# bhavyageethika/multimodal_autonomous_driving_perception_and_planning

Hardware: AMD Instinct MI355X
Metric: end-to-end frames/sec (1280x720 synthetic) (higher is better)
Workload: dtype f64; 1 GPU; config4: 64 stream(s)/GPU x 1-frame window per step, 1280x720, simulated detection + IoU tracker + 6-state KF + 21-candidate planner, one launch per step, up to 4 consecutive steps in flight; streams_per_gpu=64, window=1, graph=False, taggers=False, allgather_track_tables=False, fused_step=True, overlapped_steps=4, steps_per_library_call=8, parallelism=stream-sharded x1

## Files before the change

multimodal_autonomous_driving_perception_and_planning_amd/csrc/common.h:

```cpp
#pragma once
#include <hip/hip_runtime.h>

#include <cstdarg>
#include <cstdio>
#include <vector>

#include "avhot.h"

struct PlannerTables;

struct av_ctx {
    int device = -1;
    int n_cus = 256;
    hipStream_t side = nullptr;
    hipEvent_t ev_fork = nullptr, ev_join = nullptr;
    bool planner_ready = false;
    av_planner_cfg pcfg{};
    int n_points = 0, n_lat = 0, n_cand = 0;
    double* d_ptab = nullptr;
    double* d_cdf = nullptr;
    void* d_simtab = nullptr;
    std::vector<hipGraphExec_t> graphs;
    void* lane = nullptr;
    void* yolo = nullptr;
};

void av_set_error(const char* fmt, ...);

#define AV_HIP(expr)                                                                          \
    do {                                                                                      \
        hipError_t e_ = (expr);                                                               \
        if (e_ != hipSuccess) {                                                               \
            av_set_error("%s:%d: %s -> %s", __FILE__, __LINE__, #expr, hipGetErrorString(e_)); \
            return AV_EHIP;                                                                   \
// ... 136 lines not shown
```

multimodal_autonomous_driving_perception_and_planning_amd/csrc/planner.hip:

```cpp
#include "common.h"

#include <cmath>



namespace {

struct PlanParams {
    int n, n_lat, C;
    double dt, H;
    double w_lat, w_vel, w_acc, w_curv;
    const double *t, *alpha, *q, *dtd, *lat;
    double atq[20];
};

static const double ATAN_Q[20] = {
    -0x1.5555555555549p-2, 0x1.99999999979b9p-3,  -0x1.24924923e22b4p-3, 0x1.c71c718e5a102p-4,
    -0x1.745d120df88fbp-4, 0x1.3b1362fc35ab5p-4,  -0x1.110deef367776p-4, 0x1.e1b3c8d50e91fp-5,
    -0x1.ae2c7119eb922p-5, 0x1.81fdd2525246ap-5,  -0x1.56daf4786fd80p-5, 0x1.2575526b2309ap-5,
    -0x1.d168e01adf666p-6, 0x1.462cc26bda000p-6,  -0x1.8055065b73333p-7, 0x1.693bd6b79999ap-8,
    -0x1.fdf4e15cccccdp-10, 0x1.f224118000000p-12, -0x1.2568700000000p-14, 0x1.2ed799999999ap-18,
};

__device__ __forceinline__ double atan2_fast(double y, double x, const double (&Q)[20]) {
// ... 83 lines not shown
}
__device__ __forceinline__ void rank_and_store(const double* cc, int C, int c, int f, double* __restrict__ cost,
                                               int32_t* __restrict__ order) {
    const double mine = cc[c];
    int rank = 0;
    for (int o2 = 0; o2 < C; ++o2) {
        const double v = cc[o2];
        rank += (v < mine || (v == mine && o2 < c)) ? 1 : 0;
    }
    cost[(size_t)f * C + c] = mine;
    order[(size_t)f * C + rank] = c;
}

struct PlanNoHook {
    __device__ __forceinline__ void operator()(int) const {}
};

struct PlanLists {
    const double* ref; int n_ref;
    const double* obs; int n_obs;
};
struct PlanShared {
    static constexpr int OSTRIDE = 3;
    static constexpr bool MOVING = false;
    const double* ref; int n_ref;
    const double* obs; int n_obs;
    __device__ __forceinline__ PlanLists at(int) const { return PlanLists{ref, n_ref, obs, n_obs}; }
    __device__ __forceinline__ bool has_ref(int) const { return n_ref > 0; }
};
template <int OS>
struct PlanEachT {
// ... 14 lines not shown
            const int pth = f / ref_stride;
            l.n_ref = path_points(pth);
            l.ref = ref + (size_t)pth * rcap * 2;
        }
        if (obs) {
            const int k = n_obs[f];
            l.n_obs = k < 0 ? 0 : (k > ocap ? ocap : k);
            l.obs = obs + (size_t)f * ocap * OS;
        }
        return l;
    }
};
using PlanEach = PlanEachT<3>;
using PlanEachMoving = PlanEachT<5>;

template <int G, int NW, class Hook = PlanNoHook, class Lists = PlanShared>
__device__ __forceinline__ void plan_block_lists(const PlanParams& p, int f0, int n_states, const double* __restrict__ state,
                                                 const Lists lists, double* __restrict__ wp, double* __restrict__ cost,
                                                 int32_t* __restrict__ order, double* sm, int state_f0 = -1, int rot = 0,
                                                 Hook after1 = Hook()) {
    const int n = p.n, C = p.C;
    const int sd = state_f0 < 0 ? 0 : state_f0 - f0;
    double* vs = sm;
    double* base = vs + (size_t)G * 3 * n * 2;
    double* trig = base + even_up(G * 3 * 3);
    double* costs = trig + G * 8;
    double* stage_all = costs + 3 * even_up(G * C);
    const int CS = even_up(G * C);

    const int tid = threadIdx.x, lane = tid & 63;
    double* stage = stage_all + (size_t)(tid >> 6) * n * 6;
    const int wid = ((tid >> 6) + NW - rot) % NW;
    constexpr int P = G * 3;
    static_assert(NW >= 2, "the heading terms take the last wave");

    auto bcast = [&](double x, int i) {
        const unsigned lo = (unsigned)__builtin_amdgcn_readlane((int)(unsigned)__double_as_longlong(x), i);
        const unsigned hi = (unsigned)__builtin_amdgcn_readlane((int)(unsigned)((unsigned long long)__double_as_longlong(x) >> 32), i);
        return __longlong_as_double((long long)(((unsigned long long)hi << 32) | lo));
    };
    auto terms = [&](double v0, double dv, int i, double& v, double& vdt, double& velt, double& acct) {
        v = blend_velocity(v0, dv, p.alpha[i]);
        vdt = v * p.dt;
        velt = velocity_term(p.w_vel, v);
        acct = 0.0;
        if (i > 0)
            acct = acceleration_term(p.w_acc, v, blend_velocity(v0, dv, p.alpha[i - 1]), p.dtd[i]);
    };
    auto cost_chains = [&](double velt, double acct, unsigned long long hasm, double* b) {
        double sv = 0.0;
#pragma unroll
        for (int i = 0; i < 64; ++i)
            if (i < n) sv = sv + bcast(velt, i);
        double run = sv, sa = 0.0;
#pragma unroll
        for (int i = 1; i < 64; ++i)
            if (i < n && ((hasm >> i) & 1ull)) {
                const double term = bcast(acct, i);
                run = run + term, sa = sa + term;
            }
        if (lane == 0) b[0] = sv, b[1] = sa, b[2] = run;
    };

    const bool fast = n <= 64 && P <= NW;
    double k_velt = 0.0, k_acct = 0.0;
    unsigned long long k_has = 0;
    bool k_live = false;
    if (fast) {
        if (wid < P) {
            const int g = wid / 3, k = wid - g * 3, f = f0 + g;
            if (f < n_states) {
                const double v0 = state[(size_t)(f + sd) * 4 + 3];
                const double dv = target_speed(k) - v0;
                double* o = vs + ((size_t)(g * 3 + k) * n) * 2;
                double v = 0.0, vdt = 0.0;
                bool has = false;
                if (lane < n) terms(v0, dv, lane, v, vdt, k_velt, k_acct), has = lane > 0 && p.dtd[lane] > 0.0;
                k_has = __ballot(has), k_live = true;
                double sacc = 0.0, my_s = 0.0;
#pragma unroll
                for (int i = 1; i < 64; ++i)
                    if (i < n) {
                        sacc = sacc + bcast(vdt, i);
                        my_s = lane == i ? sacc : my_s;
                    }
                if (lane < n) o[2 * lane] = v, o[2 * lane + 1] = my_s;
            }
        }
    } else {
        for (int pr = wid; pr < P; pr += NW) {
            const int g = pr / 3, k = pr - g * 3, f = f0 + g;
            if (f >= n_states) continue;
// ... 7 lines not shown
                terms(v0, dv, i, v, vdt, velt, acct);
                o[2 * i] = v, tv[i] = vdt, tv[n + i] = velt, tv[2 * n + i] = acct;
            }
            wave_lds_fence();
            if (lane == 0) {
                double sacc = 0.0, sv = 0.0;
                o[1] = 0.0;
                sv = sv + tv[n];
                for (int i = 1; i < n; ++i) {
                    sacc = sacc + tv[i];
                    o[2 * i + 1] = sacc;
                    sv = sv + tv[n + i];
                }
                double run = sv, sa = 0.0;
                for (int i = 1; i < n; ++i) {
                    if (p.dtd[i] > 0.0) {
                        const double term = tv[2 * n + i];
                        run = run + term, sa = sa + term;
                    }
                }
                b[0] = sv, b[1] = sa, b[2] = run;
            }
            wave_lds_fence();
        }
    }
    if (wid == NW - 1 && lane < 2 * G) {
        const int g = lane >> 1, f = f0 + g;
        if (f < n_states) {
            const double h0 = state[(size_t)(f + sd) * 4 + 2];
            double* tg = trig + g * 8;
            double sn, cs;
            if (lane & 1) {
                sincos(h0 + 1.5707963267948966, &sn, &cs);
                tg[4] = cs, tg[5] = sn;
            } else {
                sincos(h0, &sn, &cs);
                tg[0] = state[(size_t)(f + sd) * 4 + 0], tg[1] = state[(size_t)(f + sd) * 4 + 1];
                tg[2] = cs, tg[3] = sn, tg[6] = h0;
            }
        }
    }
    __syncthreads();
    if (k_live) cost_chains(k_velt, k_acct, k_has, base + wid * 3);
    after1(wid);

    const double q_l = lane < n ? p.q[lane] : 0.0, q_l1 = lane + 1 < n ? p.q[lane + 1] : 0.0, t_l = lane < n ? p.t[lane] : 0.0;
    for (int j = fast ? (wid - P % NW + NW) % NW : wid; j < G * C; j += NW) {
        const int g = j / C, c = j - g * C, f = f0 + g;
        if (f >= n_states) continue;
        const PlanLists ls = lists.at(f);
        const double* ref = ls.ref;
        const double* obs = ls.obs;
        const int n_ref = ls.n_ref, n_obs = ls.n_obs;
        const bool extra = n_ref > 0 || n_obs > 0;
        const int li = c / 3, k = c - li * 3;
        const double df = p.lat[li];
        const double* tg = trig + g * 8;
        const PlanFrame fr{tg[0], tg[1], tg[2], tg[3], tg[4], tg[5]};
        const double h0 = tg[6];
        const double* o = vs + ((size_t)(g * 3 + k) * n) * 2;

        for (int i = lane; i < n; i += 64) {
            const double v = o[2 * i], s = o[2 * i + 1];
            const bool first = i == lane;
            double x, y, hd = 0.0;
            fr.point(s, df * (first ? q_l : p.q[i]), x, y);
            if (i < n - 1) {
                double x1, y1;
                fr.point(o[2 * i + 3], df * (first ? q_l1 : p.q[i + 1]), x1, y1);
                hd = atan2_fast(y1 - y, x1 - x, p.atq);
            }
            double* w = stage + (size_t)i * 6;
            w[0] = x, w[1] = y, w[2] = hd, w[3] = v, w[4] = first ? t_l : p.t[i], w[5] = 0.0;
        }
        wave_lds_fence();
        double lat_sum = 0.0, curv_sum = 0.0, obs_sum = 0.0;
        for (int i = lane; i < n; i += 64) {
            double* w = stage + (size_t)i * 6;
            double curv = 0.0;
            if (i > 0 && i < n - 1) w[5] = curv = tile_curvature(stage, i, p.dt);
            curv_sum += p.w_curv * (curv * curv);
            const double x = w[0], y = w[1];
            if (n_ref > 0) lat_sum += ref_path_term(p.w_lat, ref, n_ref, x, y);
            for (int q = 0; q < n_obs; ++q)
                add_obstacle_penalty<Lists::MOVING>(obs_sum, obs + Lists::OSTRIDE * q, x, y, w[4]);
        }
        wave_lds_fence();
        if (lane == 0) tile_last_heading(stage, n, h0);
        curv_sum = wave_sum_dpp(curv_sum);
        if (extra) lat_sum = wave_sum_dpp(lat_sum), obs_sum = wave_sum_dpp(obs_sum);
        if (lane == 0) costs[g * C + c] = lat_sum, costs[CS + g * C + c] = curv_sum, costs[2 * CS + g * C + c] = obs_sum;
        wave_lds_fence();
        if (wp) {
            const double2* src = reinterpret_cast<const double2*>(stage);
            double2* dst = reinterpret_cast<double2*>(wp + ((size_t)f * C + c) * n * 6);
            for (int q = lane; q < n * 3; q += 64) dst[q] = src[q];
        }
        wave_lds_fence();
    }
    __syncthreads();

    for (int idx = tid; idx < G * C; idx += NW * 64) {
        const int g = idx / C, c = idx - g * C, k = c % 3;
        const double* b = base + (g * 3 + k) * 3;
        const bool with_ref = lists.has_ref(f0 + g < n_states ? f0 + g : f0);
        const double va = with_ref ? (costs[idx] + b[0]) + b[1] : b[2];
        const double total = (va + costs[CS + idx]) + costs[2 * CS + idx];
        costs[idx] = total;
    }
    __syncthreads();
    for (int idx = tid; idx < G * C; idx += NW * 64) {
        const int g = idx / C, c = idx - g * C, f = f0 + g;
        if (f >= n_states) continue;
        rank_and_store(costs + g * C, C, c, f, cost, order);
    }
}

template <int G, int NW, class Hook = PlanNoHook>
__device__ __forceinline__ void plan_block(const PlanParams& p, int f0, int n_states, const double* state, const double* ref, int n_ref,
                                           const double* obs, int n_obs, double* wp, double* cost, int32_t* order, double* sm,
                                           int state_f0 = -1, int rot = 0, Hook after1 = Hook()) {
    plan_block_lists<G, NW, Hook, PlanShared>(p, f0, n_states, state, PlanShared{ref, n_ref, obs, n_obs}, wp, cost, order, sm, state_f0,
                                              rot, after1);
}

template <int G, int NW, class Lists = PlanShared>
__global__ void __launch_bounds__(NW * 64) planner_kernel(PlanParams p, int n_states, const double* __restrict__ state, Lists lists,
                                                          double* __restrict__ wp, double* __restrict__ cost,
                                                          int32_t* __restrict__ order) {
    extern __shared__ __attribute__((aligned(16))) double sm[];
    plan_block_lists<G, NW, PlanNoHook, Lists>(p, blockIdx.x * G, n_states, state, lists, wp, cost, order, sm);
}

template <int FPW, bool EXTRA, class Lists = PlanShared>
__global__ void __launch_bounds__(256) planner_wave_kernel(PlanParams p, int n_states,
                                                           const double* __restrict__ state, Lists lists,
                                                           double* __restrict__ wp, double* __restrict__ cost,
                                                           int32_t* __restrict__ order) {
// ... 476 lines not shown
```

multimodal_autonomous_driving_perception_and_planning_amd/csrc/step.hip:

```cpp
#define AVHOT_DEVICE_ONLY
#include "simdet.hip"
#include "tracker.hip"
#include "kf.hip"
#include "planner.hip"
#undef AVHOT_DEVICE_ONLY

namespace {

struct StepArgs {
    int S, h, w, dcap, tcap;
    av_tracker_cfg tcfg;
    av_kf_cfg kcfg;
    PlanParams pp;
    int32_t* frame_count; const SimRow* tab; const double* cdf;
    int32_t *det_n, *det_box, *det_cls; double* det_conf; int32_t* det_status;
    unsigned char* trk_state; av_track_row* snap; int32_t* snap_n; int32_t* det2trk;
    const double* z; double *kf_state, *vstate, *plan_state;
    double *wp, *cost; int32_t* order;
    uint8_t* wire; int stream0, frame0;
    int* flags; int seq, spin, fence, stage_off;
};

constexpr int STEP_NW = 8;

// ... 9 lines not shown
        if (!on) return;
        const unsigned long long n = __builtin_amdgcn_s_memrealtime();
        atomicAdd(acc + k, n - t);
        t = n;
    }
};

__device__ void StepClock::start(const StepArgs& a, int role) {
    on = a.flags && (a.fence & 8) && threadIdx.x == 0;
    if (!on) return;
    acc = reinterpret_cast<unsigned long long*>(a.flags + flag_stats(a.S)) + role * 16;
    t = __builtin_amdgcn_s_memrealtime();
    atomicAdd(acc + 15, 1ull);
}

__device__ __forceinline__ bool seq_enter(const StepArgs& a, int slot, int* go) {
    if (threadIdx.x == 0) {
        int ok = 0;
        int* const counter = a.flags + 32 * slot;
        int* const fault = a.flags + flag_fault(a.S);
        const int want = a.seq, spin = a.spin;
        for (int n = 0; n <= spin; ++n) {
            if ((int)((unsigned)__hip_atomic_load(counter, __ATOMIC_RELAXED, __HIP_MEMORY_SCOPE_AGENT) - (unsigned)want) >= 0) { ok = 1; break; }
            if ((n & 255) == 255 && __hip_atomic_load(fault, __ATOMIC_RELAXED, __HIP_MEMORY_SCOPE_AGENT) != 0) break;
        }
        if (!ok) atomicOr(a.flags + flag_fault(a.S), 1);
        if (ok && (a.fence & 8) && a.seq != 0) {
            const unsigned long long tp = __hip_atomic_load(reinterpret_cast<unsigned long long*>(a.flags + 32 * slot + 2), __ATOMIC_RELAXED,
                                                            __HIP_MEMORY_SCOPE_AGENT);
            const unsigned long long now = __builtin_amdgcn_s_memrealtime();
// ... 10 lines not shown
__device__ __forceinline__ void seq_leave(const StepArgs& a, int slot) {
    if (a.fence & 2) __builtin_amdgcn_fence(__ATOMIC_RELEASE, "agent");
    if (a.fence & 8)
        __hip_atomic_store(reinterpret_cast<unsigned long long*>(a.flags + 32 * slot + 2), __builtin_amdgcn_s_memrealtime(), __ATOMIC_RELAXED,
                           __HIP_MEMORY_SCOPE_AGENT);
    __hip_atomic_store(a.flags + 32 * slot, (int)((unsigned)a.seq + 1u), __ATOMIC_RELAXED, __HIP_MEMORY_SCOPE_AGENT);
}
__device__ __forceinline__ void fetch_record(const void* src, void* dst_lds, int n8, int first, int end, bool coherent) {
    unsigned long long* g = const_cast<unsigned long long*>(reinterpret_cast<const unsigned long long*>(src));
    unsigned long long* l = reinterpret_cast<unsigned long long*>(dst_lds);
    if ((int)threadIdx.x < first || (int)threadIdx.x >= end) return;
    for (int i = (int)threadIdx.x - first; i < n8; i += end - first)
        l[i] = coherent ? __hip_atomic_load(g + i, __ATOMIC_RELAXED, __HIP_MEMORY_SCOPE_AGENT) : g[i];
}

template <int PW>
__global__ void __launch_bounds__(PW * 64) hot_step_kernel(StepArgs a) {
    extern __shared__ __attribute__((aligned(16))) unsigned char smem[];
    __shared__ int go, fc_stage;
    __shared__ __attribute__((aligned(16))) double kf_stage[AV_KF_STATE_DOUBLES + 2];
    __shared__ __attribute__((aligned(32))) double kf_start[4];
    __shared__ __attribute__((aligned(16))) double kf_carry[KF_CARRY_DOUBLES];
    __shared__ int kf_tail;
    __shared__ __attribute__((aligned(16))) int d_box[8 * 4];
    __shared__ __attribute__((aligned(16))) double d_conf[8], d_area[8], z_stage[4];
    __shared__ int d_cls[8], d_n[1];
    const int tid = threadIdx.x;
    const bool seq = a.flags != nullptr;
    if ((int)blockIdx.x < a.S) {
        if (PW > STEP_NW && tid >= STEP_NW * 64) return;
        const int s = blockIdx.x;
        StepClock ck;
        ck.start(a, 0);
        int fc_before = 0;
        if (tid == 0) {
            fc_before = seq ? (int)((unsigned)a.flags[flag_base(a.S) + s] + (unsigned)a.seq) : a.frame_count[s];
            fc_stage = fc_before;
            simdet_frame<true>(0, 0, 0, a.h, a.w, a.dcap, &fc_stage, a.tab, a.cdf, d_n, d_box, d_cls, d_conf,
                               a.det_status ? a.det_status + s : nullptr);
            for (int i = 0; i < a.dcap; ++i)
                d_area[i] = (double)(d_box[4 * i + 2] - d_box[4 * i]) * (double)(d_box[4 * i + 3] - d_box[4 * i + 1]);
        }
        ck.mark(0);
        if (seq && !seq_enter(a, 2 * s, &go)) return;
        ck.mark(1);
        unsigned char* stage = smem + a.stage_off;
        int fc0 = 0;
        if (seq && tid == 0) fc0 = __hip_atomic_load(a.frame_count + s, __ATOMIC_RELAXED, __HIP_MEMORY_SCOPE_AGENT);
        fetch_record(a.trk_state + (size_t)s * state_bytes(a.tcap, a.tcfg.trajectory_length), stage,
                     (HDR_INTS * 4 + a.tcap * (int)sizeof(av_track_row)) / 8, 64, STEP_NW * 64, seq);
        if (tid == 0) {
            if (seq) {
                if (fc0 != fc_before) atomicOr(a.flags + flag_fault(a.S), 2);
                __hip_atomic_store(a.frame_count + s, fc_stage, __ATOMIC_RELAXED, __HIP_MEMORY_SCOPE_AGENT);
            } else {
                a.frame_count[s] = fc_stage;
            }
        }
        if (seq) __builtin_amdgcn_s_waitcnt(0x0F70);
        __syncthreads();
        ck.mark(2);
        if (tid < a.dcap) {
            reinterpret_cast<int4*>(a.det_box)[(size_t)s * a.dcap + tid] = reinterpret_cast<const int4*>(d_box)[tid];
            a.det_cls[(size_t)s * a.dcap + tid] = d_cls[tid];
            a.det_conf[(size_t)s * a.dcap + tid] = d_conf[tid];
            if (tid == 0) a.det_n[s] = d_n[0];
        }
        tracker_body<false, 8, STEP_NW>(a.tcfg, 1, a.dcap, d_n, d_box, d_cls, d_conf, a.tcap, a.trk_state, a.snap, a.snap_n,
                                        a.det2trk, 1, s, smem, 0xFEDCBA9876543210ull, stage, seq, 0,
                                        seq ? a.flags + 32 * (2 * s) : nullptr, (int)((unsigned)a.seq + 1u), (a.fence & 8) != 0, d_area);
        ck.mark(3);
        if (a.wire) {
            __syncthreads();
            if (tid < a.tcap)
                wire_put(a.wire + (size_t)s * (AV_WIRE_HDR_BYTES + (size_t)a.tcap * AV_WIRE_ROW_BYTES), tid, a.snap_n[s], a.tcap,
                         a.snap + (size_t)s * a.tcap, a.stream0 + s, a.frame0 + fc_stage);
        }
    } else {
        const int s = blockIdx.x - a.S;
        StepClock ck;
        ck.start(a, 1);
        if (tid < 4) z_stage[tid] = a.z[(size_t)s * 4 + tid];
        if (seq && !seq_enter(a, 2 * s + 1, &go)) return;
        ck.mark(1);
        double *vs = a.vstate + (size_t)s * AV_VSTATE_DOUBLES, *ps = a.plan_state + (size_t)s * 4;
        if (tid < 64) {
            double* rec = a.kf_state + (size_t)s * AV_KF_STATE_DOUBLES;
            fetch_record(rec, kf_stage, AV_KF_STATE_DOUBLES, 0, 64, seq);
            __builtin_amdgcn_fence(__ATOMIC_RELEASE, "workgroup", "local");
            __builtin_amdgcn_wave_barrier();
            __builtin_amdgcn_fence(__ATOMIC_ACQUIRE, "workgroup", "local");
            ck.mark(2);
            const bool separable = kf_axis_chain1(a.kcfg, z_stage, kf_stage, kf_start, kf_carry, tid);
            if (tid == 0) {
                kf_tail = separable;
                if (!separable) {
                    kf_dense_stream_lds(a.kcfg, 0, 1, z_stage, nullptr, kf_stage, vs, kf_start);
                    *reinterpret_cast<double4*>(ps) = *reinterpret_cast<const double4*>(kf_start);
                }
            }
            __builtin_amdgcn_fence(__ATOMIC_RELEASE, "workgroup", "local");
            __builtin_amdgcn_wave_barrier();
            __builtin_amdgcn_fence(__ATOMIC_ACQUIRE, "workgroup", "local");
            if (tid < AV_KF_STATE_DOUBLES) {
                if (seq)
                    __hip_atomic_store(reinterpret_cast<unsigned long long*>(rec) + tid, (unsigned long long)__double_as_longlong(kf_stage[tid]),
                                       __ATOMIC_RELAXED, __HIP_MEMORY_SCOPE_AGENT);
                else
                    rec[tid] = kf_stage[tid];
            }
        }
        ck.mark(3);
        __syncthreads();
        ck.mark(4);
        constexpr int KF_ROT = 4;
        static_assert(KF_ROT + 3 < PW, "wave 0 must not be a phase-1 pair wave nor the heading wave (task wave PW - 1)");
        if (seq && tid < 64) {
            __builtin_amdgcn_s_waitcnt(0x0F70);
            if (tid == 0) seq_leave(a, 2 * s + 1);
        }
        ck.mark(5);
        const bool clocks = seq && (a.fence & 8);
        auto tail = [&](int task_wave) {
            if (task_wave != 0 || !kf_tail) return;
            const unsigned long long t0 = clocks ? __builtin_amdgcn_s_memrealtime() : 0ull;
            kf_axis_tail1(a.kcfg, kf_stage, kf_carry, vs, ps, tid & 63);
            if (clocks && (tid & 63) == 0)
                atomicAdd(reinterpret_cast<unsigned long long*>(a.flags + flag_stats(a.S)) + 16 + 7, __builtin_amdgcn_s_memrealtime() - t0);
        };
        plan_block<1, PW>(a.pp, s, a.S, kf_start, nullptr, 0, nullptr, 0, a.wp, a.cost, a.order, reinterpret_cast<double*>(smem), 0, KF_ROT,
                          tail);
        ck.mark(6);
    }
}

}

static size_t hot_step_tracker_lds(int dcap, int tcap, int& stage_off) {
    static_assert(STEP_NW == 8, "tracker_lds_bytes sizes the replica kernel's eight column waves");
    const size_t lds_t = (tracker_lds_bytes(tcap, dcap, 1, true, 0) + 15) & ~size_t(15);
    stage_off = (int)lds_t;
    return lds_t + HDR_INTS * 4 + (size_t)tcap * sizeof(av_track_row);
}

static size_t hot_step_static_lds(const void* kernel) {
    hipFuncAttributes fa{};
    return hipFuncGetAttributes(&fa, kernel) == hipSuccess ? (size_t)fa.sharedSizeBytes : (size_t)16384;
}

static int hot_step_shape(const av_ctx* ctx, int n_streams, size_t lds_t, int depth, size_t& lds_out, int& pw_out) {
    static const size_t lds_static16 = hot_step_static_lds(reinterpret_cast<const void*>(hot_step_kernel<16>));
    static const size_t lds_static8 = hot_step_static_lds(reinterpret_cast<const void*>(hot_step_kernel<8>));
    const char* pwe = getenv("AVHOT_STEP_PW");
    int pw = pwe && atoi(pwe) == 8 ? 8 : 16;
    size_t lds = 0;
    for (;;) {
        const size_t lds_p = plan_lds_doubles(1, ctx->n_points, ctx->n_cand, pw) * 8;
        lds = lds_t > lds_p ? lds_t : lds_p;
        const size_t lds_static = pw == 16 ? lds_static16 : lds_static8;
        if (lds + lds_static > 64 * 1024) {
            AV_REQUIRE(pw == 16 && !pwe, AV_EINVAL,
                       "av_hot_step: configuration needs %zu B of dynamic + %zu B of static LDS (limit 65536)", lds, lds_static);
            pw = 8;
            continue;
        }
        if (depth <= 1) break;
        int per_cu = 0;
        if (pw == 16) AV_HIP(hipOccupancyMaxActiveBlocksPerMultiprocessor(&per_cu, hot_step_kernel<16>, 16 * 64, lds));
        else AV_HIP(hipOccupancyMaxActiveBlocksPerMultiprocessor(&per_cu, hot_step_kernel<8>, 8 * 64, lds));
        if ((long long)depth * 2 * n_streams <= (long long)per_cu * ctx->n_cus) break;
        AV_REQUIRE(pw == 16 && !pwe, AV_EINVAL, "av_hot_step: %d launches of %d workgroups in flight do not fit the device (%d per CU x %d CUs)",
                   depth, 2 * n_streams, per_cu, ctx->n_cus);
        pw = 8;
    }
    lds_out = lds, pw_out = pw;
    return AV_OK;
}

static int hot_step_args(av_ctx* ctx, const av_tracker_cfg* tcfg, const av_kf_cfg* kcfg, int n_streams, int h,
                           int w, int dcap, int tcap, int32_t* frame_count, int32_t* det_n, int32_t* det_box, int32_t* det_cls,
                           double* det_conf, int32_t* det_status, void* tracker_state, av_track_row* snap, int32_t* snap_n,
                           int32_t* det2trk, const double* z, double* kf_state, double* vstate, double* plan_state,
                           double* waypoints, double* cost, int32_t* order, void* wire, int stream0, int frame0, int32_t* seq_flags,
                           int seq, StepArgs& a, size_t& lds_out, int& pw_out, int depth = 1) {
    AV_REQUIRE(ctx && tcfg && kcfg && frame_count && det_n && det_box && det_cls && det_conf && tracker_state && z && kf_state &&
                   vstate && plan_state && cost && order,
               AV_EINVAL, "av_hot_step: null argument");
    AV_REQUIRE(n_streams > 0, AV_EINVAL, "av_hot_step: n_streams must be > 0");
    AV_REQUIRE(ctx->planner_ready && ctx->d_simtab, AV_ESTATE, "av_hot_step: call av_planner_configure first");
    AV_REQUIRE((snap == nullptr) == (snap_n == nullptr), AV_EINVAL, "av_hot_step: snap and snap_n go together");
    AV_REQUIRE(!wire || snap, AV_EINVAL, "av_hot_step: the wire tables are made from the snapshot rows");
    AV_REQUIRE(tcap == 64 && dcap >= 7 && dcap <= 8 && tcfg->iou_threshold > 0.0 && tcfg->trajectory_length >= 1, AV_EINVAL,
               "av_hot_step: needs tcap 64, dcap 7..8 and iou_threshold > 0 (use the stage calls otherwise)");
    AV_REQUIRE(h > 0 && w > 121, AV_EINVAL, "av_hot_step: frame %dx%d too small", w, h);
    a = StepArgs{};
    a.S = n_streams, a.h = h, a.w = w, a.dcap = dcap, a.tcap = tcap;
    a.tcfg = *tcfg, a.kcfg = *kcfg;
    fill_params(ctx, a.pp);
    a.frame_count = frame_count, a.tab = (const SimRow*)ctx->d_simtab, a.cdf = ctx->d_cdf;
    a.det_n = det_n, a.det_box = det_box, a.det_cls = det_cls, a.det_conf = det_conf, a.det_status = det_status;
    a.trk_state = (unsigned char*)tracker_state, a.snap = snap, a.snap_n = snap_n, a.det2trk = det2trk;
    a.z = z, a.kf_state = kf_state, a.vstate = vstate, a.plan_state = plan_state;
    a.wp = waypoints, a.cost = cost, a.order = order;
    a.wire = (uint8_t*)wire, a.stream0 = stream0, a.frame0 = frame0;
    a.flags = seq_flags, a.seq = seq;
    const char* spe = seq_flags ? getenv("AVHOT_STEP_SPIN") : nullptr;
    a.spin = spe ? atoi(spe) : (1 << 22);
    const char* fe = seq_flags ? getenv("AVHOT_STEP_FENCE") : nullptr;
    a.fence = fe ? atoi(fe) : 0;
    int stage_off = 0;
    const size_t lds_t = hot_step_tracker_lds(dcap, tcap, stage_off);
    a.stage_off = stage_off;
    return hot_step_shape(ctx, n_streams, lds_t, depth, lds_out, pw_out);
}

static int hot_step_go(const StepArgs& a, size_t lds, int pw, av_stream_t stream) {
    if (pw == 16) hipLaunchKernelGGL(hot_step_kernel<16>, dim3(2 * a.S), dim3(16 * 64), lds, as_stream(stream), a);
    else hipLaunchKernelGGL(hot_step_kernel<8>, dim3(2 * a.S), dim3(8 * 64), lds, as_stream(stream), a);
    AV_LAUNCH_CHECK();
    return AV_OK;
}

static int hot_step_launch(av_ctx* ctx, av_stream_t stream, const av_tracker_cfg* tcfg, const av_kf_cfg* kcfg, int n_streams, int h,
                           int w, int dcap, int tcap, int32_t* frame_count, int32_t* det_n, int32_t* det_box, int32_t* det_cls,
                           double* det_conf, int32_t* det_status, void* tracker_state, av_track_row* snap, int32_t* snap_n,
                           int32_t* det2trk, const double* z, double* kf_state, double* vstate, double* plan_state,
                           double* waypoints, double* cost, int32_t* order, void* wire, int stream0, int frame0, int32_t* seq_flags,
                           int seq, int depth = 1) {
    StepArgs a;
    size_t lds;
    int pw;
    const int rc = hot_step_args(ctx, tcfg, kcfg, n_streams, h, w, dcap, tcap, frame_count, det_n, det_box, det_cls, det_conf, det_status,
                                 tracker_state, snap, snap_n, det2trk, z, kf_state, vstate, plan_state, waypoints, cost, order, wire, stream0,
                                 frame0, seq_flags, seq, a, lds, pw, depth);
    return rc != AV_OK ? rc : hot_step_go(a, lds, pw, stream);
}

extern "C" int av_hot_step_fits(av_ctx* ctx, int n_streams, int dcap, int tcap, int depth) {
    AV_REQUIRE(ctx && n_streams > 0 && depth >= 1, AV_EINVAL, "av_hot_step_fits: bad argument");
    AV_REQUIRE(ctx->planner_ready, AV_ESTATE, "av_hot_step_fits: call av_planner_configure first");
    AV_REQUIRE(tcap == 64 && dcap >= 7 && dcap <= 8, AV_EINVAL, "av_hot_step_fits: needs tcap 64, dcap 7..8");
    AV_HIP(hipSetDevice(ctx->device));
    int stage_off = 0;
    size_t lds = 0;
    int pw = 0;
    return hot_step_shape(ctx, n_streams, hot_step_tracker_lds(dcap, tcap, stage_off), depth, lds, pw);
}

extern "C" int av_hot_step(av_ctx* ctx, av_stream_t stream, const av_tracker_cfg* tcfg, const av_kf_cfg* kcfg, int n_streams, int h,
                           int w, int dcap, int tcap, int32_t* frame_count, int32_t* det_n, int32_t* det_box, int32_t* det_cls,
                           double* det_conf, int32_t* det_status, void* tracker_state, av_track_row* snap, int32_t* snap_n,
                           int32_t* det2trk, const double* z, double* kf_state, double* vstate, double* plan_state,
                           double* waypoints, double* cost, int32_t* order, void* wire, int stream0, int frame0) {
    return hot_step_launch(ctx, stream, tcfg, kcfg, n_streams, h, w, dcap, tcap, frame_count, det_n, det_box, det_cls, det_conf, det_status,
                           tracker_state, snap, snap_n, det2trk, z, kf_state, vstate, plan_state, waypoints, cost, order, wire, stream0,
                           frame0, nullptr, 0);
}

extern "C" int av_hot_step_seq(av_ctx* ctx, av_stream_t stream, const av_tracker_cfg* tcfg, const av_kf_cfg* kcfg, int n_streams, int h,
                               int w, int dcap, int tcap, int32_t* frame_count, int32_t* det_n, int32_t* det_box, int32_t* det_cls,
                               double* det_conf, int32_t* det_status, void* tracker_state, av_track_row* snap, int32_t* snap_n,
// ... 7 lines not shown
                           frame0, seq_flags, seq, depth);
}

extern "C" int av_hot_steps_seq(av_ctx* ctx, int depth, const av_stream_t* streams, const av_tracker_cfg* tcfg, const av_kf_cfg* kcfg,
                                int n_streams, int h, int w, int dcap, int tcap, int32_t* frame_count, int32_t* det_status,
                                void* tracker_state, double* kf_state, const av_step_set* sets, const double* z_steps, void* wire_steps,
                                int stream0, int frame0, int32_t* seq_flags, int seq0, int n_steps) {
    AV_REQUIRE(seq_flags && n_steps > 0 && sets && streams, AV_EINVAL, "av_hot_steps_seq: bad argument");
    AV_REQUIRE(depth >= 2 && depth <= AV_STEP_MAX_DEPTH, AV_EINVAL, "av_hot_steps_seq: depth %d not in [2, %d]", depth, AV_STEP_MAX_DEPTH);
    for (int k = 0; k < depth; ++k)
        for (int j = 0; j < k; ++j)
            AV_REQUIRE(streams[k] != streams[j], AV_EINVAL, "av_hot_steps_seq: the %d steps in flight need %d different HIP streams", depth, depth);
    StepArgs par[AV_STEP_MAX_DEPTH];
    size_t lds = 0;
    int pw = 16;
    for (int k = 0; k < depth; ++k) {
        const av_step_set& b = sets[k];
        const int rc = hot_step_args(ctx, tcfg, kcfg, n_streams, h, w, dcap, tcap, frame_count, b.det_n, b.det_box, b.det_cls, b.det_conf, det_status,
                                     tracker_state, b.snap, b.snap_n, b.det2trk, z_steps ? z_steps : b.z, kf_state, b.vstate, b.plan_state,
                                     b.waypoints, b.cost, b.order, wire_steps, stream0, frame0, seq_flags, seq0, par[k], lds, pw, depth);
        if (rc != AV_OK) return rc;
    }
    const size_t zb = (size_t)n_streams * 4, wb = (size_t)n_streams * (AV_WIRE_HDR_BYTES + (size_t)tcap * AV_WIRE_ROW_BYTES);
    for (int i = 0; i < n_steps; ++i) {
        const int q = (int)((unsigned)seq0 + (unsigned)i), k = (int)((unsigned)q % (unsigned)depth);
        StepArgs& a = par[k];
        a.seq = q;
        if (z_steps) a.z = z_steps + (size_t)i * zb;
        if (wire_steps) a.wire = (uint8_t*)wire_steps + (size_t)i * wb;
        const int rc = hot_step_go(a, lds, pw, streams[k]);
        if (rc != AV_OK) return rc;
    }
    return AV_OK;
}
```

Baseline: 13.36 million frames/s.

## Stage planner tables in LDS, specialize step kernel on sequencing, cache launch shape

The fused step kernel gains template parameters for sequenced mode and for keeping the planner lookup tables (t, alpha, q, dtd, lat) in LDS. Idle waves copy the tables into shared memory while wave 0 waits on the sequence gate, and kernel arguments are pinned into scalar registers across the spin-wait. The host now caches the computed launch shape in the context so occupancy queries are not repeated on every launch. The intent is to remove repeated global table reads and per-launch host overhead, at the cost of more LDS per block, more kernel instantiations, and a risk of lower occupancy.

```diff
diff --git a/multimodal_autonomous_driving_perception_and_planning_amd/csrc/common.h b/multimodal_autonomous_driving_perception_and_planning_amd/csrc/common.h
--- a/multimodal_autonomous_driving_perception_and_planning_amd/csrc/common.h
+++ b/multimodal_autonomous_driving_perception_and_planning_amd/csrc/common.h
@@ -18,6 +18,13 @@
     av_planner_cfg pcfg{};
     int n_points = 0, n_lat = 0, n_cand = 0;
     double* d_ptab = nullptr;
+    struct StepShape {
+        bool valid = false;
+        int n = 0, C = 0, n_lat = 0, S = 0, depth = 0, pw_env = 0;
+        size_t lds_t = 0, lds = 0;
+        int pw = 0;
+        bool tab = false;
+    } step_shape;
     double* d_cdf = nullptr;
     void* d_simtab = nullptr;
     std::vector<hipGraphExec_t> graphs;
diff --git a/multimodal_autonomous_driving_perception_and_planning_amd/csrc/planner.hip b/multimodal_autonomous_driving_perception_and_planning_amd/csrc/planner.hip
--- a/multimodal_autonomous_driving_perception_and_planning_amd/csrc/planner.hip
+++ b/multimodal_autonomous_driving_perception_and_planning_amd/csrc/planner.hip
@@ -121,7 +121,9 @@
 
 struct PlanNoHook {
     __device__ __forceinline__ void operator()(int) const {}
-};
+    __device__ __forceinline__ void mark(int) const {}
+};
+enum { PLAN_MARK_PHASE1 = 0, PLAN_MARK_CHAINS = 1, PLAN_MARK_PHASE2 = 2, PLAN_MARK_TRAJ = 3 };
 
 struct PlanLists {
     const double* ref; int n_ref;
@@ -166,11 +168,28 @@
 using PlanEach = PlanEachT<3>;
 using PlanEachMoving = PlanEachT<5>;
 
-template <int G, int NW, class Hook = PlanNoHook, class Lists = PlanShared>
+struct PlanTabGlobal {
+    __device__ __forceinline__ double t(const PlanParams& p, int i) const { return p.t[i]; }
+    __device__ __forceinline__ double alpha(const PlanParams& p, int i) const { return p.alpha[i]; }
+    __device__ __forceinline__ double q(const PlanParams& p, int i) const { return p.q[i]; }
+    __device__ __forceinline__ double dtd(const PlanParams& p, int i) const { return p.dtd[i]; }
+    __device__ __forceinline__ double lat(const PlanParams& p, int li) const { return p.lat[li]; }
+};
+__host__ __device__ inline size_t plan_tab_doubles(int n, int n_lat) { return (size_t)4 * n + n_lat; }
+struct PlanTabLds {
+    const double* tab;
+    __device__ __forceinline__ double t(const PlanParams&, int i) const { return tab[i]; }
+    __device__ __forceinline__ double alpha(const PlanParams& p, int i) const { return tab[p.n + i]; }
+    __device__ __forceinline__ double q(const PlanParams& p, int i) const { return tab[2 * p.n + i]; }
+    __device__ __forceinline__ double dtd(const PlanParams& p, int i) const { return tab[3 * p.n + i]; }
+    __device__ __forceinline__ double lat(const PlanParams& p, int li) const { return tab[4 * p.n + li]; }
+};
+
+template <int G, int NW, class Hook = PlanNoHook, class Lists = PlanShared, class Tab = PlanTabGlobal>
 __device__ __forceinline__ void plan_block_lists(const PlanParams& p, int f0, int n_states, const double* __restrict__ state,
                                                  const Lists lists, double* __restrict__ wp, double* __restrict__ cost,
                                                  int32_t* __restrict__ order, double* sm, int state_f0 = -1, int rot = 0,
-                                                 Hook after1 = Hook()) {
+                                                 Hook after1 = Hook(), const Tab tab = Tab()) {
     const int n = p.n, C = p.C;
     const int sd = state_f0 < 0 ? 0 : state_f0 - f0;
     double* vs = sm;
@@ -192,12 +211,12 @@
         return __longlong_as_double((long long)(((unsigned long long)hi << 32) | lo));
     };
     auto terms = [&](double v0, double dv, int i, double& v, double& vdt, double& velt, double& acct) {
-        v = blend_velocity(v0, dv, p.alpha[i]);
+        v = blend_velocity(v0, dv, tab.alpha(p, i));
         vdt = v * p.dt;
         velt = velocity_term(p.w_vel, v);
         acct = 0.0;
         if (i > 0)
-            acct = acceleration_term(p.w_acc, v, blend_velocity(v0, dv, p.alpha[i - 1]), p.dtd[i]);
+            acct = acceleration_term(p.w_acc, v, blend_velocity(v0, dv, tab.alpha(p, i - 1)), tab.dtd(p, i));
     };
     auto cost_chains = [&](double velt, double acct, unsigned long long hasm, double* b) {
         double sv = 0.0;
@@ -227,7 +246,7 @@
                 double* o = vs + ((size_t)(g * 3 + k) * n) * 2;
                 double v = 0.0, vdt = 0.0;
                 bool has = false;
-                if (lane < n) terms(v0, dv, lane, v, vdt, k_velt, k_acct), has = lane > 0 && p.dtd[lane] > 0.0;
+                if (lane < n) terms(v0, dv, lane, v, vdt, k_velt, k_acct), has = lane > 0 && tab.dtd(p, lane) > 0.0;
                 k_has = __ballot(has), k_live = true;
                 double sacc = 0.0, my_s = 0.0;
 #pragma unroll
@@ -265,7 +284,7 @@
                 }
                 double run = sv, sa = 0.0;
                 for (int i = 1; i < n; ++i) {
-                    if (p.dtd[i] > 0.0) {
+                    if (tab.dtd(p, i) > 0.0) {
                         const double term = tv[2 * n + i];
                         run = run + term, sa = sa + term;
                     }
@@ -291,12 +310,16 @@
             }
         }
     }
+    after1.mark(PLAN_MARK_PHASE1);
     __syncthreads();
     if (k_live) cost_chains(k_velt, k_acct, k_has, base + wid * 3);
     after1(wid);
 
-    const double q_l = lane < n ? p.q[lane] : 0.0, q_l1 = lane + 1 < n ? p.q[lane + 1] : 0.0, t_l = lane < n ? p.t[lane] : 0.0;
-    for (int j = fast ? (wid - P % NW + NW) % NW : wid; j < G * C; j += NW) {
+    const double q_l = lane < n ? tab.q(p, lane) : 0.0, q_l1 = lane + 1 < n ? tab.q(p, lane + 1) : 0.0;
+    const double t_l = lane < n ? tab.t(p, lane) : 0.0;
+    after1.mark(PLAN_MARK_CHAINS);
+    int turn = 0;
+    for (int j = fast ? (wid - P % NW + NW) % NW : wid; j < G * C; j += NW, ++turn) {
         const int g = j / C, c = j - g * C, f = f0 + g;
         if (f >= n_states) continue;
         const PlanLists ls = lists.at(f);
@@ -305,7 +328,7 @@
         const int n_ref = ls.n_ref, n_obs = ls.n_obs;
         const bool extra = n_ref > 0 || n_obs > 0;
         const int li = c / 3, k = c - li * 3;
-        const double df = p.lat[li];
+        const double df = tab.lat(p, li);
         const double* tg = trig + g * 8;
         const PlanFrame fr{tg[0], tg[1], tg[2], tg[3], tg[4], tg[5]};
         const double h0 = tg[6];
@@ -315,14 +338,14 @@
             const double v = o[2 * i], s = o[2 * i + 1];
             const bool first = i == lane;
             double x, y, hd = 0.0;
-            fr.point(s, df * (first ? q_l : p.q[i]), x, y);
+            fr.point(s, df * (first ? q_l : tab.q(p, i)), x, y);
             if (i < n - 1) {
                 double x1, y1;
-                fr.point(o[2 * i + 3], df * (first ? q_l1 : p.q[i + 1]), x1, y1);
+                fr.point(o[2 * i + 3], df * (first ? q_l1 : tab.q(p, i + 1)), x1, y1);
                 hd = atan2_fast(y1 - y, x1 - x, p.atq);
             }
             double* w = stage + (size_t)i * 6;
-            w[0] = x, w[1] = y, w[2] = hd, w[3] = v, w[4] = first ? t_l : p.t[i], w[5] = 0.0;
+            w[0] = x, w[1] = y, w[2] = hd, w[3] = v, w[4] = first ? t_l : tab.t(p, i), w[5] = 0.0;
         }
         wave_lds_fence();
         double lat_sum = 0.0, curv_sum = 0.0, obs_sum = 0.0;
@@ -348,8 +371,10 @@
             for (int q = lane; q < n * 3; q += 64) dst[q] = src[q];
         }
         wave_lds_fence();
+        after1.mark(PLAN_MARK_TRAJ + turn);
     }
     __syncthreads();
+    after1.mark(PLAN_MARK_PHASE2);
 
     for (int idx = tid; idx < G * C; idx += NW * 64) {
         const int g = idx / C, c = idx - g * C, k = c % 3;
@@ -367,12 +392,12 @@
     }
 }
 
-template <int G, int NW, class Hook = PlanNoHook>
+template <int G, int NW, class Hook = PlanNoHook, class Tab = PlanTabGlobal>
 __device__ __forceinline__ void plan_block(const PlanParams& p, int f0, int n_states, const double* state, const double* ref, int n_ref,
                                            const double* obs, int n_obs, double* wp, double* cost, int32_t* order, double* sm,
-                                           int state_f0 = -1, int rot = 0, Hook after1 = Hook()) {
-    plan_block_lists<G, NW, Hook, PlanShared>(p, f0, n_states, state, PlanShared{ref, n_ref, obs, n_obs}, wp, cost, order, sm, state_f0,
-                                              rot, after1);
+                                           int state_f0 = -1, int rot = 0, Hook after1 = Hook(), const Tab tab = Tab()) {
+    plan_block_lists<G, NW, Hook, PlanShared, Tab>(p, f0, n_states, state, PlanShared{ref, n_ref, obs, n_obs}, wp, cost, order, sm,
+                                                   state_f0, rot, after1, tab);
 }
 
 template <int G, int NW, class Lists = PlanShared>
diff --git a/multimodal_autonomous_driving_perception_and_planning_amd/csrc/step.hip b/multimodal_autonomous_driving_perception_and_planning_amd/csrc/step.hip
--- a/multimodal_autonomous_driving_perception_and_planning_amd/csrc/step.hip
+++ b/multimodal_autonomous_driving_perception_and_planning_amd/csrc/step.hip
@@ -47,6 +47,32 @@
     atomicAdd(acc + 15, 1ull);
 }
 
+template <class T>
+__device__ __forceinline__ void pin(T& x) {
+    asm volatile("" : "+s"(x));
+}
+template <class T>
+__device__ __forceinline__ void pin(T*& x) {
+    auto g = (__attribute__((address_space(1))) T*)x;
+    asm volatile("" : "+s"(g));
+    x = (T*)g;
+}
+template <class T, class... Ts>
+__device__ __forceinline__ void pin(T& x, Ts&... more) {
+    pin(x), pin(more...);
+}
+
+__device__ __forceinline__ int plan_mark_slot(int k) {
+    return k == PLAN_MARK_PHASE1 ? 10 : k == PLAN_MARK_CHAINS ? 11 : k == PLAN_MARK_PHASE2 ? 0 : 12 + (k - PLAN_MARK_TRAJ < 2 ? k - PLAN_MARK_TRAJ : 2);
+}
+template <class Tail>
+struct StepPlanHook {
+    Tail tail;
+    StepClock& ck;
+    __device__ __forceinline__ void operator()(int task_wave) const { tail(task_wave); }
+    __device__ __forceinline__ void mark(int k) const { ck.mark(plan_mark_slot(k)); }
+};
+
 __device__ __forceinline__ bool seq_enter(const StepArgs& a, int slot, int* go) {
     if (threadIdx.x == 0) {
         int ok = 0;
@@ -87,7 +113,7 @@
         l[i] = coherent ? __hip_atomic_load(g + i, __ATOMIC_RELAXED, __HIP_MEMORY_SCOPE_AGENT) : g[i];
 }
 
-template <int PW>
+template <int PW, bool TAB_LDS, bool SEQ>
 __global__ void __launch_bounds__(PW * 64) hot_step_kernel(StepArgs a) {
     extern __shared__ __attribute__((aligned(16))) unsigned char smem[];
     __shared__ int go, fc_stage;
@@ -99,76 +125,95 @@
     __shared__ __attribute__((aligned(16))) double d_conf[8], d_area[8], z_stage[4];
     __shared__ int d_cls[8], d_n[1];
     const int tid = threadIdx.x;
-    const bool seq = a.flags != nullptr;
+    constexpr bool seq = SEQ;
     if ((int)blockIdx.x < a.S) {
         if (PW > STEP_NW && tid >= STEP_NW * 64) return;
         const int s = blockIdx.x;
+        StepArgs b = a;
         StepClock ck;
-        ck.start(a, 0);
+        if constexpr (SEQ) ck.start(b, 0);
+        else ck.on = false;
         int fc_before = 0;
         if (tid == 0) {
-            fc_before = seq ? (int)((unsigned)a.flags[flag_base(a.S) + s] + (unsigned)a.seq) : a.frame_count[s];
+            fc_before = seq ? (int)((unsigned)b.flags[flag_base(b.S) + s] + (unsigned)b.seq) : b.frame_count[s];
             fc_stage = fc_before;
-            simdet_frame<true>(0, 0, 0, a.h, a.w, a.dcap, &fc_stage, a.tab, a.cdf, d_n, d_box, d_cls, d_conf,
-                               a.det_status ? a.det_status + s : nullptr);
-            for (int i = 0; i < a.dcap; ++i)
+            simdet_frame<true>(0, 0, 0, b.h, b.w, b.dcap, &fc_stage, b.tab, b.cdf, d_n, d_box, d_cls, d_conf,
+                               b.det_status ? b.det_status + s : nullptr);
+            for (int i = 0; i < b.dcap; ++i)
                 d_area[i] = (double)(d_box[4 * i + 2] - d_box[4 * i]) * (double)(d_box[4 * i + 3] - d_box[4 * i + 1]);
         }
         ck.mark(0);
-        if (seq && !seq_enter(a, 2 * s, &go)) return;
+        if constexpr (SEQ)
+            pin(b.S, b.dcap, b.tcap, b.tcfg.iou_threshold, b.tcfg.max_age, b.tcfg.min_hits, b.tcfg.trajectory_length, b.frame_count, b.det_n,
+                b.det_box, b.det_cls, b.det_conf, b.trk_state, b.snap, b.snap_n, b.det2trk, b.wire, b.stream0, b.frame0, b.flags, b.seq, b.spin,
+                b.fence, b.stage_off);
+        if (seq && !seq_enter(b, 2 * s, &go)) return;
         ck.mark(1);
-        unsigned char* stage = smem + a.stage_off;
+        unsigned char* stage = smem + b.stage_off;
         int fc0 = 0;
-        if (seq && tid == 0) fc0 = __hip_atomic_load(a.frame_count + s, __ATOMIC_RELAXED, __HIP_MEMORY_SCOPE_AGENT);
-        fetch_record(a.trk_state + (size_t)s * state_bytes(a.tcap, a.tcfg.trajectory_length), stage,
-                     (HDR_INTS * 4 + a.tcap * (int)sizeof(av_track_row)) / 8, 64, STEP_NW * 64, seq);
+        if (seq && tid == 0) fc0 = __hip_atomic_load(b.frame_count + s, __ATOMIC_RELAXED, __HIP_MEMORY_SCOPE_AGENT);
+        fetch_record(b.trk_state + (size_t)s * state_bytes(b.tcap, b.tcfg.trajectory_length), stage,
+                     (HDR_INTS * 4 + b.tcap * (int)sizeof(av_track_row)) / 8, 64, STEP_NW * 64, seq);
         if (tid == 0) {
             if (seq) {
-                if (fc0 != fc_before) atomicOr(a.flags + flag_fault(a.S), 2);
-                __hip_atomic_store(a.frame_count + s, fc_stage, __ATOMIC_RELAXED, __HIP_MEMORY_SCOPE_AGENT);
+                if (fc0 != fc_before) atomicOr(b.flags + flag_fault(b.S), 2);
+                __hip_atomic_store(b.frame_count + s, fc_stage, __ATOMIC_RELAXED, __HIP_MEMORY_SCOPE_AGENT);
             } else {
-                a.frame_count[s] = fc_stage;
+                b.frame_count[s] = fc_stage;
             }
         }
         if (seq) __builtin_amdgcn_s_waitcnt(0x0F70);
         __syncthreads();
         ck.mark(2);
-        if (tid < a.dcap) {
-            reinterpret_cast<int4*>(a.det_box)[(size_t)s * a.dcap + tid] = reinterpret_cast<const int4*>(d_box)[tid];
-            a.det_cls[(size_t)s * a.dcap + tid] = d_cls[tid];
-            a.det_conf[(size_t)s * a.dcap + tid] = d_conf[tid];
-            if (tid == 0) a.det_n[s] = d_n[0];
-        }
-        tracker_body<false, 8, STEP_NW>(a.tcfg, 1, a.dcap, d_n, d_box, d_cls, d_conf, a.tcap, a.trk_state, a.snap, a.snap_n,
-                                        a.det2trk, 1, s, smem, 0xFEDCBA9876543210ull, stage, seq, 0,
-                                        seq ? a.flags + 32 * (2 * s) : nullptr, (int)((unsigned)a.seq + 1u), (a.fence & 8) != 0, d_area);
+        if (tid < b.dcap) {
+            reinterpret_cast<int4*>(b.det_box)[(size_t)s * b.dcap + tid] = reinterpret_cast<const int4*>(d_box)[tid];
+            b.det_cls[(size_t)s * b.dcap + tid] = d_cls[tid];
+            b.det_conf[(size_t)s * b.dcap + tid] = d_conf[tid];
+            if (tid == 0) b.det_n[s] = d_n[0];
+        }
+        tracker_body<false, 8, STEP_NW>(b.tcfg, 1, b.dcap, d_n, d_box, d_cls, d_conf, b.tcap, b.trk_state, b.snap, b.snap_n,
+                                        b.det2trk, 1, s, smem, 0xFEDCBA9876543210ull, stage, seq, 0,
+                                        seq ? b.flags + 32 * (2 * s) : nullptr, (int)((unsigned)b.seq + 1u), (b.fence & 8) != 0, d_area);
         ck.mark(3);
-        if (a.wire) {
+        if (b.wire) {
             __syncthreads();
-            if (tid < a.tcap)
-                wire_put(a.wire + (size_t)s * (AV_WIRE_HDR_BYTES + (size_t)a.tcap * AV_WIRE_ROW_BYTES), tid, a.snap_n[s], a.tcap,
-                         a.snap + (size_t)s * a.tcap, a.stream0 + s, a.frame0 + fc_stage);
+            if (tid < b.tcap)
+                wire_put(b.wire + (size_t)s * (AV_WIRE_HDR_BYTES + (size_t)b.tcap * AV_WIRE_ROW_BYTES), tid, b.snap_n[s], b.tcap,
+                         b.snap + (size_t)s * b.tcap, b.stream0 + s, b.frame0 + fc_stage);
         }
     } else {
         const int s = blockIdx.x - a.S;
+        StepArgs b = a;
         StepClock ck;
-        ck.start(a, 1);
-        if (tid < 4) z_stage[tid] = a.z[(size_t)s * 4 + tid];
-        if (seq && !seq_enter(a, 2 * s + 1, &go)) return;
+        if constexpr (SEQ) ck.start(b, 1);
+        else ck.on = false;
+        if (tid < 4) z_stage[tid] = b.z[(size_t)s * 4 + tid];
+        double* const ptab = reinterpret_cast<double*>(smem) + plan_lds_doubles(1, b.pp.n, b.pp.C, PW);
+        if (TAB_LDS && tid >= 64)
+            for (int i = tid - 64, nt = (int)plan_tab_doubles(b.pp.n, b.pp.n_lat); i < nt; i += (PW - 1) * 64) ptab[i] = b.pp.t[i];
+        if constexpr (SEQ) {
+            pin(b.S, b.kcfg.dt, b.kcfg.process_noise, b.kcfg.measurement_noise, b.kf_state, b.vstate, b.plan_state, b.wp, b.cost, b.order,
+                b.flags, b.seq, b.spin, b.fence);
+            pin(b.pp.n, b.pp.n_lat, b.pp.C, b.pp.dt, b.pp.w_lat, b.pp.w_vel, b.pp.w_acc, b.pp.w_curv);
+            if (!TAB_LDS) pin(b.pp.t, b.pp.alpha, b.pp.q, b.pp.dtd, b.pp.lat);
+#pragma unroll
+            for (int k = 0; k < 20; ++k) pin(b.pp.atq[k]);
+        }
+        if (seq && !seq_enter(b, 2 * s + 1, &go)) return;
         ck.mark(1);
-        double *vs = a.vstate + (size_t)s * AV_VSTATE_DOUBLES, *ps = a.plan_state + (size_t)s * 4;
+        double *vs = b.vstate + (size_t)s * AV_VSTATE_DOUBLES, *ps = b.plan_state + (size_t)s * 4;
         if (tid < 64) {
-            double* rec = a.kf_state + (size_t)s * AV_KF_STATE_DOUBLES;
+            double* rec = b.kf_state + (size_t)s * AV_KF_STATE_DOUBLES;
             fetch_record(rec, kf_stage, AV_KF_STATE_DOUBLES, 0, 64, seq);
             __builtin_amdgcn_fence(__ATOMIC_RELEASE, "workgroup", "local");
             __builtin_amdgcn_wave_barrier();
             __builtin_amdgcn_fence(__ATOMIC_ACQUIRE, "workgroup", "local");
             ck.mark(2);
-            const bool separable = kf_axis_chain1(a.kcfg, z_stage, kf_stage, kf_start, kf_carry, tid);
+            const bool separable = kf_axis_chain1(b.kcfg, z_stage, kf_stage, kf_start, kf_carry, tid);
             if (tid == 0) {
                 kf_tail = separable;
                 if (!separable) {
-                    kf_dense_stream_lds(a.kcfg, 0, 1, z_stage, nullptr, kf_stage, vs, kf_start);
+                    kf_dense_stream_lds(b.kcfg, 0, 1, z_stage, nullptr, kf_stage, vs, kf_start);
                     *reinterpret_cast<double4*>(ps) = *reinterpret_cast<const double4*>(kf_start);
                 }
             }
@@ -190,19 +235,24 @@
         static_assert(KF_ROT + 3 < PW, "wave 0 must not be a phase-1 pair wave nor the heading wave (task wave PW - 1)");
         if (seq && tid < 64) {
             __builtin_amdgcn_s_waitcnt(0x0F70);
-            if (tid == 0) seq_leave(a, 2 * s + 1);
+            if (tid == 0) seq_leave(b, 2 * s + 1);
         }
         ck.mark(5);
-        const bool clocks = seq && (a.fence & 8);
+        const bool clocks = seq && (b.fence & 8);
         auto tail = [&](int task_wave) {
             if (task_wave != 0 || !kf_tail) return;
             const unsigned long long t0 = clocks ? __builtin_amdgcn_s_memrealtime() : 0ull;
-            kf_axis_tail1(a.kcfg, kf_stage, kf_carry, vs, ps, tid & 63);
+            kf_axis_tail1(b.kcfg, kf_stage, kf_carry, vs, ps, tid & 63);
             if (clocks && (tid & 63) == 0)
-                atomicAdd(reinterpret_cast<unsigned long long*>(a.flags + flag_stats(a.S)) + 16 + 7, __builtin_amdgcn_s_memrealtime() - t0);
+                atomicAdd(reinterpret_cast<unsigned long long*>(b.flags + flag_stats(b.S)) + 16 + 7, __builtin_amdgcn_s_memrealtime() - t0);
         };
-        plan_block<1, PW>(a.pp, s, a.S, kf_start, nullptr, 0, nullptr, 0, a.wp, a.cost, a.order, reinterpret_cast<double*>(smem), 0, KF_ROT,
-                          tail);
+        const StepPlanHook<decltype(tail)> hook{tail, ck};
+        if constexpr (TAB_LDS)
+            plan_block<1, PW>(b.pp, s, b.S, kf_start, nullptr, 0, nullptr, 0, b.wp, b.cost, b.order, reinterpret_cast<double*>(smem), 0,
+                              KF_ROT, hook, PlanTabLds{ptab});
+        else
+            plan_block<1, PW>(b.pp, s, b.S, kf_start, nullptr, 0, nullptr, 0, b.wp, b.cost, b.order, reinterpret_cast<double*>(smem), 0,
+                              KF_ROT, hook);
         ck.mark(6);
     }
 }
@@ -216,21 +266,45 @@
     return lds_t + HDR_INTS * 4 + (size_t)tcap * sizeof(av_track_row);
 }
 
-static size_t hot_step_static_lds(const void* kernel) {
-    hipFuncAttributes fa{};
-    return hipFuncGetAttributes(&fa, kernel) == hipSuccess ? (size_t)fa.sharedSizeBytes : (size_t)16384;
-}
-
-static int hot_step_shape(const av_ctx* ctx, int n_streams, size_t lds_t, int depth, size_t& lds_out, int& pw_out) {
-    static const size_t lds_static16 = hot_step_static_lds(reinterpret_cast<const void*>(hot_step_kernel<16>));
-    static const size_t lds_static8 = hot_step_static_lds(reinterpret_cast<const void*>(hot_step_kernel<8>));
+using StepKernel = void (*)(StepArgs);
+static StepKernel hot_step_fn(int pw, bool tab, bool seq) {
+    if (pw == 16) return !seq ? hot_step_kernel<16, false, false> : tab ? hot_step_kernel<16, true, true> : hot_step_kernel<16, false, true>;
+    return !seq ? hot_step_kernel<8, false, false> : tab ? hot_step_kernel<8, true, true> : hot_step_kernel<8, false, true>;
+}
+
+static size_t hot_step_static_lds(int pw, bool tab, bool seq) {
+    struct Known {
+        size_t v[2][2][2];
+        Known() {
+            for (int p = 0; p < 2; ++p)
+                for (int t = 0; t < 2; ++t)
+                    for (int q = 0; q < 2; ++q) {
+                        hipFuncAttributes fa{};
+                        const bool ok = hipFuncGetAttributes(&fa, reinterpret_cast<const void*>(hot_step_fn(p ? 16 : 8, t, q))) == hipSuccess;
+                        v[p][t][q] = ok ? (size_t)fa.sharedSizeBytes : (size_t)16384;
+                    }
+        }
+    };
+    static const Known known;
+    return known.v[pw == 16][tab][seq];
+}
+
+static int hot_step_shape(av_ctx* ctx, int n_streams, size_t lds_t, int depth, size_t& lds_out, int& pw_out, bool& tab_out) {
     const char* pwe = getenv("AVHOT_STEP_PW");
-    int pw = pwe && atoi(pwe) == 8 ? 8 : 16;
+    const int pw_env = pwe ? atoi(pwe) : 0;
+    av_ctx::StepShape& k = ctx->step_shape;
+    if (k.valid && k.n == ctx->n_points && k.C == ctx->n_cand && k.n_lat == ctx->n_lat && k.S == n_streams && k.depth == depth &&
+        k.pw_env == pw_env && k.lds_t == lds_t) {
+        lds_out = k.lds, pw_out = k.pw, tab_out = k.tab;
+        return AV_OK;
+    }
+    const bool seq = depth > 1;
+    int pw = pwe && pw_env == 8 ? 8 : 16;
     size_t lds = 0;
     for (;;) {
         const size_t lds_p = plan_lds_doubles(1, ctx->n_points, ctx->n_cand, pw) * 8;
         lds = lds_t > lds_p ? lds_t : lds_p;
-        const size_t lds_static = pw == 16 ? lds_static16 : lds_static8;
+        const size_t lds_static = hot_step_static_lds(pw, false, seq);
         if (lds + lds_static > 64 * 1024) {
             AV_REQUIRE(pw == 16 && !pwe, AV_EINVAL,
                        "av_hot_step: configuration needs %zu B of dynamic + %zu B of static LDS (limit 65536)", lds, lds_static);
@@ -239,14 +313,22 @@
         }
         if (depth <= 1) break;
         int per_cu = 0;
-        if (pw == 16) AV_HIP(hipOccupancyMaxActiveBlocksPerMultiprocessor(&per_cu, hot_step_kernel<16>, 16 * 64, lds));
-        else AV_HIP(hipOccupancyMaxActiveBlocksPerMultiprocessor(&per_cu, hot_step_kernel<8>, 8 * 64, lds));
+        AV_HIP(hipOccupancyMaxActiveBlocksPerMultiprocessor(&per_cu, hot_step_fn(pw, false, seq), pw * 64, lds));
         if ((long long)depth * 2 * n_streams <= (long long)per_cu * ctx->n_cus) break;
         AV_REQUIRE(pw == 16 && !pwe, AV_EINVAL, "av_hot_step: %d launches of %d workgroups in flight do not fit the device (%d per CU x %d CUs)",
                    depth, 2 * n_streams, per_cu, ctx->n_cus);
         pw = 8;
     }
-    lds_out = lds, pw_out = pw;
+    const size_t lds_p = (plan_lds_doubles(1, ctx->n_points, ctx->n_cand, pw) + plan_tab_doubles(ctx->n_points, ctx->n_lat)) * 8;
+    const size_t lds_tab = lds_t > lds_p ? lds_t : lds_p;
+    bool tab = seq && lds_tab + hot_step_static_lds(pw, true, seq) <= 64 * 1024;
+    if (tab) {
+        int per_cu = 0;
+        AV_HIP(hipOccupancyMaxActiveBlocksPerMultiprocessor(&per_cu, hot_step_fn(pw, true, seq), pw * 64, lds_tab));
+        tab = (long long)depth * 2 * n_streams <= (long long)per_cu * ctx->n_cus;
+    }
+    lds_out = tab ? lds_tab : lds, pw_out = pw, tab_out = tab;
+    k = av_ctx::StepShape{true, ctx->n_points, ctx->n_cand, ctx->n_lat, n_streams, depth, pw_env, lds_t, lds_out, pw, tab};
     return AV_OK;
 }
 
@@ -255,7 +337,7 @@
                            double* det_conf, int32_t* det_status, void* tracker_state, av_track_row* snap, int32_t* snap_n,
                            int32_t* det2trk, const double* z, double* kf_state, double* vstate, double* plan_state,
                            double* waypoints, double* cost, int32_t* order, void* wire, int stream0, int frame0, int32_t* seq_flags,
-                           int seq, StepArgs& a, size_t& lds_out, int& pw_out, int depth = 1) {
+                           int seq, StepArgs& a, size_t& lds_out, int& pw_out, bool& tab_out, int depth = 1) {
     AV_REQUIRE(ctx && tcfg && kcfg && frame_count && det_n && det_box && det_cls && det_conf && tracker_state && z && kf_state &&
                    vstate && plan_state && cost && order,
                AV_EINVAL, "av_hot_step: null argument");
@@ -284,12 +366,11 @@
     int stage_off = 0;
     const size_t lds_t = hot_step_tracker_lds(dcap, tcap, stage_off);
     a.stage_off = stage_off;
-    return hot_step_shape(ctx, n_streams, lds_t, depth, lds_out, pw_out);
-}
-
-static int hot_step_go(const StepArgs& a, size_t lds, int pw, av_stream_t stream) {
-    if (pw == 16) hipLaunchKernelGGL(hot_step_kernel<16>, dim3(2 * a.S), dim3(16 * 64), lds, as_stream(stream), a);
-    else hipLaunchKernelGGL(hot_step_kernel<8>, dim3(2 * a.S), dim3(8 * 64), lds, as_stream(stream), a);
+    return hot_step_shape(ctx, n_streams, lds_t, depth, lds_out, pw_out, tab_out);
+}
+
+static int hot_step_go(const StepArgs& a, size_t lds, int pw, bool tab, av_stream_t stream) {
+    hipLaunchKernelGGL(hot_step_fn(pw, tab, a.flags != nullptr), dim3(2 * a.S), dim3(pw * 64), lds, as_stream(stream), a);
     AV_LAUNCH_CHECK();
     return AV_OK;
 }
@@ -303,10 +384,11 @@
     StepArgs a;
     size_t lds;
     int pw;
+    bool tab;
     const int rc = hot_step_args(ctx, tcfg, kcfg, n_streams, h, w, dcap, tcap, frame_count, det_n, det_box, det_cls, det_conf, det_status,
                                  tracker_state, snap, snap_n, det2trk, z, kf_state, vstate, plan_state, waypoints, cost, order, wire, stream0,
-                                 frame0, seq_flags, seq, a, lds, pw, depth);
-    return rc != AV_OK ? rc : hot_step_go(a, lds, pw, stream);
+                                 frame0, seq_flags, seq, a, lds, pw, tab, depth);
+    return rc != AV_OK ? rc : hot_step_go(a, lds, pw, tab, stream);
 }
 
 extern "C" int av_hot_step_fits(av_ctx* ctx, int n_streams, int dcap, int tcap, int depth) {
@@ -317,7 +399,8 @@
     int stage_off = 0;
     size_t lds = 0;
     int pw = 0;
-    return hot_step_shape(ctx, n_streams, hot_step_tracker_lds(dcap, tcap, stage_off), depth, lds, pw);
+    bool tab = false;
+    return hot_step_shape(ctx, n_streams, hot_step_tracker_lds(dcap, tcap, stage_off), depth, lds, pw, tab);
 }
 
 extern "C" int av_hot_step(av_ctx* ctx, av_stream_t stream, const av_tracker_cfg* tcfg, const av_kf_cfg* kcfg, int n_streams, int h,
@@ -355,11 +438,12 @@
     StepArgs par[AV_STEP_MAX_DEPTH];
     size_t lds = 0;
     int pw = 16;
+    bool tab = false;
     for (int k = 0; k < depth; ++k) {
         const av_step_set& b = sets[k];
         const int rc = hot_step_args(ctx, tcfg, kcfg, n_streams, h, w, dcap, tcap, frame_count, b.det_n, b.det_box, b.det_cls, b.det_conf, det_status,
                                      tracker_state, b.snap, b.snap_n, b.det2trk, z_steps ? z_steps : b.z, kf_state, b.vstate, b.plan_state,
-                                     b.waypoints, b.cost, b.order, wire_steps, stream0, frame0, seq_flags, seq0, par[k], lds, pw, depth);
+                                     b.waypoints, b.cost, b.order, wire_steps, stream0, frame0, seq_flags, seq0, par[k], lds, pw, tab, depth);
         if (rc != AV_OK) return rc;
     }
     const size_t zb = (size_t)n_streams * 4, wb = (size_t)n_streams * (AV_WIRE_HDR_BYTES + (size_t)tcap * AV_WIRE_ROW_BYTES);
@@ -369,7 +453,7 @@
         a.seq = q;
         if (z_steps) a.z = z_steps + (size_t)i * zb;
         if (wire_steps) a.wire = (uint8_t*)wire_steps + (size_t)i * wb;
-        const int rc = hot_step_go(a, lds, pw, streams[k]);
+        const int rc = hot_step_go(a, lds, pw, tab, streams[k]);
         if (rc != AV_OK) return rc;
     }
     return AV_OK;
```

Measured after the change: 13.41 million frames/s (median of 2 runs). About the same (+0.4%).
